# baowj-678/koordinator

Hardware: AMD Instinct MI355X
Metric: pods placed/sec + (pod,node) Filter+Score evals/sec at 50k nodes, 1-8 GPUs (higher is better)
Workload: dtype int64; 1 GPU; config4: 50000 nodes x 100000 pods, 30% BE, NodeResourcesFit + LoadAwareScheduling, shipped scheduler-config.yaml profile; nodes=50000, pods=100000, batch_pods=24, pipeline_lag=2, parallelism=node-shard x1

## Files before the change

### koordinator_amd/csrc/api.hip

```cpp
#include <hip/hip_runtime.h>
#include <rccl/rccl.h>

#include <algorithm>
#include <array>
#include <cmath>
#include <condition_variable>
#include <memory>
#include <mutex>
#include <cstdio>
#include <cstdlib>
#include <cstring>
#include <chrono>
#include <string>
#include <unordered_map>
#include <vector>

#include "../../include/koordhip.h"
#include "cls.h"
#include "diag.h"
#include "diag_ext.h"
#include "reasons.h"
#include "preempt.h"
#include "kernels.h"
#include "place_plan.hpp"
// ... 2541 lines not shown
  return 0;
}

int enqueue_rounds(koordhip_ctx *c, const PlaceCall &pc) {
  const kh::PlacePlan &plan = pc.plan;
  if (plan.cls) return 0;
  const int32_t P = plan.P, K = plan.K, lag = plan.lag, total = c->n_staged, lo = pc.lo, hi = pc.hi;
  const bool two = plan.two, exch = plan.exch, serial = plan.serial;
  kh::PipeSync *sync = pc.sync;
  hipStream_t rs = serial ? c->stream : c->rstream;
  for (int32_t r = 0; r < plan.rounds; r++) {
    const int32_t p0 = r * P, np = std::min(P, total - p0);
    const int par = r & 1;
    hipStream_t es = (two && par) ? c->stream2 : c->stream;
    const int slot = two ? par : 0;
    const kh::DevPod *pods = c->d_pods + p0;
    const bool timed = r % plan.tstride == 0;
    uint64_t *lists = c->d_lists + (size_t)(r & (2 * lag - 1)) * kListBuf;
    if (r > lag && !serial) HIP_TRY(kh::launch_wait_resolved(sync, r - lag, es));
    if (exch) {
      if (np < P) HIP_TRY(hipMemsetAsync(lists, 0, (size_t)P * K * sizeof(uint64_t), es));
      if (int e = topk_batch(c, pods, np, K, lo, hi, lists, timed, nullptr, 0, es, slot)) return e;
      if (int e = exchange(c, lists, (size_t)P * K, slot, es)) return e;
      HIP_TRY(kh::launch_topk_merge(gather_buf(c, slot), K, (int64_t)P * K, np, c->world, K, c->score_bits,
                                    c->d_final + (size_t)(r & (2 * lag - 1)) * kListBuf, sync, par, es));
    } else {
      if (int e = topk_batch(c, pods, np, K, lo, hi, lists, timed, sync, par, es, slot)) return e;
    }
    if (!plan.persistent) {
      if (!serial) {
        HIP_TRY(hipEventRecord(c->ev_res[r % kRing], c->stream));
        HIP_TRY(hipStreamWaitEvent(rs, c->ev_res[r % kRing], 0));
      }
      int32_t tm = -1;
      if (int e = timed_begin(c, TK_RESOLVE, rs, &tm)) return e;
      if (int e = launch_resolve_rounds(c, pc, r, r + 1, c->monotone, 1, rs)) return e;
      if (int e = timed_end(c, tm, rs)) return e;
    }
  }
  return 0;
}

int join_streams(koordhip_ctx *c, const PlaceCall &pc) {
  const kh::PlacePlan &plan = pc.plan;
  if (int e = timed_end(c, pc.res_tm, c->rstream)) return e;
  if (plan.two) {
    HIP_TRY(hipEventRecord(c->ev_eval2, c->stream2));
    HIP_TRY(hipStreamWaitEvent(c->stream, c->ev_eval2, 0));
  }
  if (plan.ext_pipe && plan.rounds > 0) {
    HIP_TRY(hipStreamWaitEvent(c->stream, c->ev_ext, 0));
    HIP_TRY(hipStreamWaitEvent(c->stream, c->ev_ext2, 0));
  }
  if (!plan.serial) {
    HIP_TRY(hipEventRecord(c->ev_res[0], c->rstream));
    HIP_TRY(hipStreamWaitEvent(c->stream, c->ev_res[0], 0));
  }
  HIP_TRY(hipEventRecord(c->t1, c->stream));
  c->pipe_check = true;
  return 0;
}

int print_stamps(koordhip_ctx *c, const kh::PlacePlan &plan) {
  if (!c->d_dbg) return 0;
  uint64_t h[64];
  HIP_TRY(hipMemcpyAsync(h, c->d_dbg, sizeof(h), hipMemcpyDeviceToHost, c->stream));
  HIP_TRY(hipStreamSynchronize(c->stream));
  if (c->eval_fused && h[40])
    std::fprintf(stderr,
                 "[koordhip stamps] k_eval_topk: %llu workgroups, cycles per workgroup: evaluate %.0f  select+emit %.0f  "
                 "publish %.0f | %llu merges, cycles per merge %.0f, candidates per merge %.1f\n",
                 (unsigned long long)h[40], (double)h[41] / h[40], (double)h[42] / h[40], (double)h[43] / h[40],
                 (unsigned long long)h[45], h[45] ? (double)h[44] / h[45] : 0.0, h[45] ? (double)h[46] / h[45] : 0.0);
  std::fprintf(stderr,
               "[koordhip stamps] resolve cycles: prologue walk %llu  hash %llu  waiting for lists %llu  loop %llu  "
               "release %llu | pods %llu  bulk commits %llu  staged pods %llu  general-path pods %llu  HBM row loads %llu\n",
               (unsigned long long)h[0], (unsigned long long)h[2], (unsigned long long)h[1], (unsigned long long)h[4],
               (unsigned long long)h[14], (unsigned long long)h[7], (unsigned long long)h[20],
               (unsigned long long)h[21], (unsigned long long)h[5], (unsigned long long)h[6]);
  std::fprintf(stderr, "[koordhip stamps] resolve loop cycles: conflict detection %llu  bulk commits %llu | "
               "general path: candidate+keys %llu  commit %llu | write-back %llu | kernel total %llu\n",
               (unsigned long long)h[16], (unsigned long long)h[17], (unsigned long long)h[18],
               (unsigned long long)h[19], (unsigned long long)h[25], (unsigned long long)h[26]);
  std::fprintf(stderr, "[koordhip stamps] round overlap: wave-0 end-of-round barrier %llu | wave 1: waiting for the "
               "next lists %llu  loading them %llu\n",
               (unsigned long long)h[29], (unsigned long long)h[27], (unsigned long long)h[28]);
  if (c->numa)
    std::fprintf(stderr, "[koordhip stamps] NUMA: accumulator replays full %llu cycles / %llu, spread %llu / %llu | "
                 "row passes of required-spread pods %llu / %llu, of other pods %llu / %llu\n",
                 (unsigned long long)h[32], (unsigned long long)h[33], (unsigned long long)h[34],
                 (unsigned long long)h[35], (unsigned long long)h[36], (unsigned long long)h[37],
                 (unsigned long long)h[38], (unsigned long long)h[39]);
  std::fprintf(stderr, "[koordhip stamps] general path detail: candidate + table keys %llu  row evaluations %llu | "
               "pods served by the key tables %llu\n",
               (unsigned long long)h[22], (unsigned long long)h[23], (unsigned long long)h[24]);
  std::fprintf(stderr, "[koordhip stamps] prologue phases: walk %llu  winner rows %llu (HBM loads %llu)  conflicts %llu | "
               "general-path causes: staged conflict %llu  slow %llu  voided by a general commit %llu\n",
               (unsigned long long)h[48], (unsigned long long)h[49], (unsigned long long)h[51],
               (unsigned long long)h[50], (unsigned long long)h[52], (unsigned long long)h[53],
               (unsigned long long)h[54]);
  std::fprintf(stderr, "[koordhip stamps] general path split: list + X + c %llu cycles | pods with ready key tables %llu | "
               "evaluation passes %llu\n",
               (unsigned long long)h[55], (unsigned long long)h[56], (unsigned long long)h[57]);
  if (plan.cls) {
    uint64_t q[32];
    HIP_TRY(hipMemcpy(q, c->d_dbg + 64, sizeof(q), hipMemcpyDeviceToHost));
    const double nl = (double)std::max<uint64_t>(q[7], 1), nc = (double)std::max<uint64_t>(q[15], 1);
    std::fprintf(stderr, "[koordhip stamps] class lists, cycles per launch (workgroup 0, %llu launches): buffer %.0f  log %.0f  "
                 "touched keys %.0f  compaction %.0f  sort %.0f  merge %.0f  outputs %.0f | builds (%llu): histogram %.0f  "
                 "fine %.0f  emit %.0f  sort %.0f  write %.0f\n", (unsigned long long)q[7], q[0] / nl, q[1] / nl, q[2] / nl,
                 q[3] / nl, q[4] / nl, q[5] / nl, q[6] / nl, (unsigned long long)q[15], q[8] / nc, q[9] / nc, q[10] / nc,
                 q[11] / nc, q[12] / nc);
  }
  {
    uint64_t q[4] = {0, 0, 0, 0}, rw[8] = {0, 0, 0, 0, 0, 0, 0, 0};
    HIP_TRY(hipMemcpy(q, c->d_dbg + 90, sizeof(q), hipMemcpyDeviceToHost));
    HIP_TRY(hipMemcpy(rw, c->d_dbg + 107, sizeof(rw), hipMemcpyDeviceToHost));
    std::fprintf(stderr, "[koordhip stamps] chain re-walks: walk + keys %llu (entries + claims %llu, row + evaluation "
                 "%llu)  winners' rows %llu cycles | winner rows loaded from HBM %llu\n", (unsigned long long)rw[0],
                 (unsigned long long)rw[5], (unsigned long long)rw[6], (unsigned long long)rw[1],
                 (unsigned long long)rw[2]);
    std::fprintf(stderr, "[koordhip stamps] chained decisions: %llu cycles, %llu pods resolved | claim tables %llu  "
                 "re-walks %llu  re-check + closure %llu  final table %llu | rounds with a lazy "
                 "claim table %llu\n", (unsigned long long)h[62],
                 (unsigned long long)h[63], (unsigned long long)q[0], (unsigned long long)q[1],
                 (unsigned long long)q[2], (unsigned long long)q[3], (unsigned long long)rw[7]);
    uint64_t sp[7] = {0, 0, 0, 0, 0, 0, 0};
    HIP_TRY(hipMemcpy(sp, c->d_dbg + 116, sizeof(sp), hipMemcpyDeviceToHost));
    std::fprintf(stderr, "[koordhip stamps] same-class speculation: made %llu  validated %llu  invalidated %llu | "
                 "given up: no head row %llu  walk past the entries %llu  winner assumed-claimed %llu  winner row in "
                 "HBM %llu\n", (unsigned long long)sp[0], (unsigned long long)sp[1], (unsigned long long)sp[2],
                 (unsigned long long)sp[3], (unsigned long long)sp[4], (unsigned long long)sp[5],
                 (unsigned long long)sp[6]);
  }
  if (plan.ext_pipe) {
    uint64_t q[8];
    HIP_TRY(hipMemcpy(q, c->d_dbg + 80, sizeof(q), hipMemcpyDeviceToHost));
    const double np = (double)std::max<uint64_t>(q[6], 1);
    std::fprintf(stderr, "[koordhip stamps] device pods (k_ext_pre / k_ext_final): %llu, resolve cycles from the "
                 "hand-off to the answer %llu (%.0f per pod) | final launch per pod: workgroup 0 evaluate + fold "
                 "%.0f | last workgroup: decide + publish %.0f  device commit %.0f\n",
                 (unsigned long long)h[31], (unsigned long long)h[30], h[31] ? (double)h[30] / h[31] : 0.0,
                 q[0] / np, q[3] / np, q[4] / np);
    uint64_t r[16];
    HIP_TRY(hipMemcpy(r, c->d_dbg + 96, sizeof(r), hipMemcpyDeviceToHost));
    std::fprintf(stderr, "[koordhip stamps] device-pod finals: workgroups with a full (device) re-evaluation %llu, "
                 "their re-evaluation %.2f us each\n", (unsigned long long)r[14], r[14] ? r[15] * 0.01 / r[14] : 0.0);
    const double nb = (double)std::max<uint64_t>(r[10], 1);
    std::fprintf(stderr, "[koordhip stamps] device-pod finals, us: request seen -> last workgroup arrived %.2f per pod | "
                 "per workgroup: -> gate seen %.2f  X marked %.2f  re-evaluated %.2f  folded + arrived %.2f\n",
                 r[5] * 0.01 / np, r[6] * 0.01 / nb, r[7] * 0.01 / nb, r[8] * 0.01 / nb, r[9] * 0.01 / nb);
    std::fprintf(stderr, "[koordhip stamps] device-pod hand-offs, us per pod: the request seen -> published %.2f | "
                 "requests already set when the final's first workgroup started: %llu of %llu | pre-evaluation "
                 "published after the request: %llu pods, waited %.2f us each\n",
                 r[2] * 0.01 / np, (unsigned long long)r[0], (unsigned long long)q[6], (unsigned long long)r[1],
                 r[1] ? r[3] * 0.01 / r[1] : 0.0);
  }
  std::fprintf(stderr, "[koordhip stamps] general commit split: row source %llu  Reserve delta %llu  voiding + "
               "outputs %llu cycles | winners already in M %llu\n",
               (unsigned long long)h[58], (unsigned long long)h[59], (unsigned long long)h[60],
               (unsigned long long)h[61]);
  return 0;
}

int place_staged_impl(koordhip_ctx *c) {
  if (!c->loaded) return fail(KOORDHIP_ESTATE, "no snapshot loaded");
  c->pipe_err = false;
  c->pipe_errc = 0;
  c->pipe_check = false;
// ... 1124 lines not shown
```

### koordinator_amd/csrc/eval.hpp

```cpp
#pragma once
#include <hip/hip_runtime.h>
#include <stdint.h>

#include "../../include/koordhip.h"
#include "numa.hpp"

namespace kh {

template <typename T>
__device__ __forceinline__ void st_wt(T *p, T v) {
  if constexpr (sizeof(T) == 8) {
    __hip_atomic_store(reinterpret_cast<uint64_t *>(p), __builtin_bit_cast(uint64_t, v), __ATOMIC_RELAXED,
                       __HIP_MEMORY_SCOPE_AGENT);
  } else if constexpr (sizeof(T) == 4) {
    __hip_atomic_store(reinterpret_cast<uint32_t *>(p), __builtin_bit_cast(uint32_t, v), __ATOMIC_RELAXED,
                       __HIP_MEMORY_SCOPE_AGENT);
  } else {
    __hip_atomic_store(reinterpret_cast<uint8_t *>(p), __builtin_bit_cast(uint8_t, v), __ATOMIC_RELAXED,
                       __HIP_MEMORY_SCOPE_AGENT);
  }
}

template <typename T>
using gptr = __attribute__((address_space(1))) T *;
// ... 573 lines not shown
  v.sa = d.sallow ? as_global(d.sallow)[i] : 0xFFFFFFFFu;
}

template <bool Z = true>
__device__ __forceinline__ void load_numa_row(NumaRow &r, const DevNodes &d, int32_t i) {
  r.cls = as_global(d.nu.node_cls)[i];
  r.nflags = as_global(d.nu.nflags)[i];
  r.cnt = as_global(d.nu.cnt)[i];
#pragma unroll
  for (int w = 0; w < NW; w++) {
    r.fr[w] = as_global(d.nu.fr[w])[i];
    r.ep[w] = as_global(d.nu.ep[w])[i];
    r.en[w] = as_global(d.nu.en[w])[i];
  }
  if (Z && d.nu.za && topo_policy(r.nflags) != 0) load_zones(r, d, i);
  r.amp = d.nu.amp ? as_global(d.nu.amp)[i] : 1.0;
}

template <bool Z = true>
__device__ __forceinline__ void store_numa_row(const NumaRow &r, const DevNodes &d, int32_t i) {
  d.nu.cnt[i] = r.cnt;
#pragma unroll
  for (int w = 0; w < NW; w++) {
    d.nu.fr[w][i] = r.fr[w];
    d.nu.ep[w][i] = r.ep[w];
    d.nu.en[w][i] = r.en[w];
  }
  if (Z && d.nu.za && topo_policy(r.nflags) != 0) {
    double *zu = d.nu.zu + (size_t)i * 2 * ZMAX;
#pragma unroll
    for (int q = 0; q < ZMAX; q++) {
      zu[q] = r.zu[0][q];
      zu[ZMAX + q] = r.zu[1][q];
    }
  }
}

__device__ __forceinline__ void numa_apply(NumaRow &r, const DevPod &p, const uint64_t *cpus, int sign,
                                           const uint64_t *P = nullptr) {
  const int ex = (int)KOORDHIP_NUMA_EXCLUSIVE(p.numa_policy);
  int n = 0;
#pragma unroll
  for (int w = 0; w < NW; w++) {
    n += __popcll(P ? (cpus[w] & ~P[w]) : cpus[w]);
    if (sign > 0) {
      r.fr[w] &= ~cpus[w];
      r.ep[w] = (r.ep[w] & ~cpus[w]) | (ex == (int)KOORDHIP_CPUEXCL_PCPU ? cpus[w] : 0ull);
      r.en[w] = (r.en[w] & ~cpus[w]) | (ex == (int)KOORDHIP_CPUEXCL_NUMA ? cpus[w] : 0ull);
    } else {
      r.fr[w] |= cpus[w];
      r.ep[w] &= ~cpus[w];
      r.en[w] &= ~cpus[w];
    }
  }
  r.cnt += sign * n;
}

__device__ __forceinline__ void store_row(const NV &v, const DevNodes &d, int32_t i) {
#pragma unroll
  for (int r = 0; r < KOORDHIP_NRES; r++) d.requested[r][i] = v.r[r];
  d.npods[i] = v.npods;
  d.nz_cpu[i] = v.nz_cpu;
  d.nz_mem[i] = v.nz_mem;
  d.la_used_cpu[i] = v.la_u_cpu;
  d.la_used_mem[i] = v.la_u_mem;
  d.la_used_prod_cpu[i] = v.la_up_cpu;
  d.la_used_prod_mem[i] = v.la_up_mem;
  d.flags[i] = (uint8_t)v.flags;
}

__device__ __forceinline__ void store_row_wt(const NV &v, const DevNodes &d, int32_t i) {
#pragma unroll
  for (int r = 0; r < KOORDHIP_NRES; r++) st_wt_g(&d.requested[r][i], v.r[r]);
  st_wt_g(&d.npods[i], v.npods);
  st_wt_g(&d.nz_cpu[i], v.nz_cpu);
  st_wt_g(&d.nz_mem[i], v.nz_mem);
  st_wt_g(&d.la_used_cpu[i], v.la_u_cpu);
  st_wt_g(&d.la_used_mem[i], v.la_u_mem);
  st_wt_g(&d.la_used_prod_cpu[i], v.la_up_cpu);
  st_wt_g(&d.la_used_prod_mem[i], v.la_up_mem);
  st_wt_g(&d.flags[i], (uint8_t)v.flags);
}

template <bool Z = true>
__device__ __forceinline__ void store_numa_row_wt(const NumaRow &r, const DevNodes &d, int32_t i) {
  st_wt_g(&d.nu.cnt[i], r.cnt);
#pragma unroll
  for (int w = 0; w < NW; w++) {
    st_wt_g(&d.nu.fr[w][i], r.fr[w]);
    st_wt_g(&d.nu.ep[w][i], r.ep[w]);
    st_wt_g(&d.nu.en[w][i], r.en[w]);
  }
  if (Z && d.nu.za && topo_policy(r.nflags) != 0) {
    double *zu = d.nu.zu + (size_t)i * 2 * ZMAX;
#pragma unroll
    for (int q = 0; q < ZMAX; q++) {
      st_wt_g(&zu[q], r.zu[0][q]);
      st_wt_g(&zu[ZMAX + q], r.zu[1][q]);
    }
  }
}

template <bool Z, bool WAVE = false>
__device__ __attribute__((noinline)) bool numa_reserve(const DevNumaClass *classes, NumaRow &row, const DevPod &pod,
                                                       uint64_t *cpus_out, const uint64_t *pref = nullptr) {
  NumaRow r = row;
  const DevPod p = pod;
  uint64_t cpus[NW] = {0, 0, 0, 0};
  uint64_t P[NW] = {0, 0, 0, 0};
  if (pref)
    for (int w = 0; w < NW; w++) P[w] = pref[w];
  for (int w = 0; w < NW; w++) cpus_out[w] = 0;
  const bool cs = (p.flags & KOORDHIP_POD_CPUSET) != 0;
  const int tp = Z ? topo_policy(r.nflags) : 0;
  if (!cs && tp == 0) return true;
  if (r.cls < 0) return false;
  const DevNumaClass &C = classes[r.cls];
  if (!Z || tp == 0) {
    if (cs && any4(P)) {
      if (!numa_allocate_pref_in<WAVE>(C, r, p, P, cpus)) return false;
    } else if (!numa_allocate_in<WAVE>(C, r, p, cpus)) {
      return false;
    }
    numa_apply(r, p, cpus, +1, P);
  } else {
    uint32_t mask;
    double av[2][ZMAX];
    zone_avail_all(r, C.nnuma, av);
    if (!zone_hint(C.nnuma, av, p, tp, &mask)) return false;
    const bool hp = cs && any4(P);
    if (hp) {
      double ru[ZMAX];
      zone_reusable(C, P, ru);
      zone_avail_reus(r, C.nnuma, ru, av);
    }
    double z[2][ZMAX];
    if (mask && !zone_alloc(C.nnuma, av, p, mask, z)) return false;
    if (cs) {
      if (mask) {
        if (!zone_allocate_in(C, r, p, z, cpus, hp ? P : nullptr)) return false;
      } else if (hp) {
        if (!numa_allocate_pref_in<WAVE>(C, r, p, P, cpus)) return false;
      } else if (!numa_allocate_in<WAVE>(C, r, p, cpus)) {
        return false;
      }
      numa_apply(r, p, cpus, +1, P);
    }
    if (mask) {
#pragma unroll
      for (int k = 0; k < ZMAX; k++) {
        r.zu[0][k] += z[0][k];
        r.zu[1][k] += z[1][k];
      }
    }
  }
  row = r;
  for (int w = 0; w < NW; w++) cpus_out[w] = cpus[w];
  return true;
}

template <int S>
__device__ __forceinline__ uint32_t filter_status(const DevCfg &c, const DevPod &pod, const NV &v,
                                                  const NumaRowRS<S> &r, const DevNumaClass *classes, int nmatch,
                                                  uint32_t mm, ResvXS rx = no_rx()) {
  uint32_t b = 0;
  if ((c.filt & KOORDHIP_PLUGIN_NODE_STATIC) && !((v.sa >> pod.sclass) & 1u)) b |= KOORDHIP_ST_STATIC_FAIL;
// ... 72 lines not shown
```

### koordinator_amd/csrc/kernels.hip

```cpp
#include <hip/hip_runtime.h>

#include <algorithm>
#include <cstdio>

#include "eval.hpp"
#include "karg.hpp"
#include "kernels.h"
#include "pipe.hpp"
#include "rows.hpp"

namespace kh {


__device__ __forceinline__ uint64_t shfl_u64(uint64_t v, int src) {
  uint32_t lo = __shfl((uint32_t)v, src, 64);
  uint32_t hi = __shfl((uint32_t)(v >> 32), src, 64);
  return ((uint64_t)hi << 32) | lo;
}
__device__ __forceinline__ uint64_t shfl_up_u64(uint64_t v, int d) {
  uint32_t lo = __shfl_up((uint32_t)v, d, 64);
  uint32_t hi = __shfl_up((uint32_t)(v >> 32), d, 64);
  return ((uint64_t)hi << 32) | lo;
}
__device__ __forceinline__ uint64_t shfl_xor_u64(uint64_t v, int m) {
// ... 1329 lines not shown
  NR *prenr2 = reinterpret_cast<NR *>(lds + ofs.pre_numa2);
  int32_t *pre_node2 = reinterpret_cast<int32_t *>(lds + ofs.pre_node2);
  __shared__ int32_t pnode[RES_MAXP_ROUND];
  __shared__ int32_t pgen[RES_MAXP_ROUND];
  __shared__ int32_t seg_w[RES_MAXP_ROUND];
  __shared__ int32_t ckey[RES_HASH], cval[RES_HASH];
  __shared__ int32_t sh_mp, sh_stop, sh_done, sh_chain;
  __shared__ uint64_t sh_rsv;
  const int t = threadIdx.x, lane = lane_id();
  const int32_t words = (n_nodes + 31) >> 5;
  const int32_t HP = max(1, RES_PRE / P);
  auto nodes = [&]() -> decltype(auto) {
    if constexpr (NM <= 2) {
      return *reinterpret_cast<const DevNodes *>(lds + ofs.ptab);
    } else {
      const DevNodes *p = dn;
      asm volatile("" : "+s"(p));
      return DevNodes(*p);
    }
  };
  if constexpr (NM <= 2) {
    constexpr int PW = (int)((NUMA ? offsetof(DevNodes, rv) : offsetof(DevNodes, nu)) / 8);
    static_assert(PW <= RES_THREADS, "one 8-byte word of the pointer table per thread");
    if (t < PW) reinterpret_cast<uint64_t *>(lds + ofs.ptab)[t] = reinterpret_cast<const uint64_t *>(dn)[t];
  }
  const bool two = kp > 64;
  const bool chain_on = (monotone & 2) && ofs.dep >= 0;
  static_assert(RES_WE == 8, "a pod's rank word: one rank byte + RES_WE - 1 predecessor bytes");
  const bool spec_on = NM == 0 && chain_on && ofs.rank >= 0 && pod_cls != nullptr && !(monotone & 16);
  uint64_t *rk = reinterpret_cast<uint64_t *>(lds + (ofs.rank >= 0 ? ofs.rank : 0));
  uint64_t *rk2 = reinterpret_cast<uint64_t *>(lds + (ofs.rank2 >= 0 ? ofs.rank2 : 0));
  const uint64_t t_kernel = (dbg && t == 0) ? stamp() : 0;
  if (t == 0) {
    sh_mp = r_begin > 0 ? min(mbuf[0], P) : 0;
    sh_stop = 0;
  }
  for (int32_t x = t; x < words; x += RES_THREADS) {
    modmap[x] = 0;
    gbits[x] = 0;
  }
  for (int32_t x = t; x < RES_MAXP_ROUND; x += RES_THREADS) {
    moved[x] = 0;
    ready[x] = 0;
  }
  for (int32_t x = t; x < RES_HASH; x += RES_THREADS) {
    ckey[x] = -1;
    cval[x] = 64;
  }
  const DevNumaClass *cls = ncls;
  if constexpr (NUMA) {
    const int32_t nc = dn->nu.ncls;
    if (nc <= NUMA_LDS_CLASSES) {
      uint4 *dst = reinterpret_cast<uint4 *>(lds + ofs.classes);
      const uint4 *src = reinterpret_cast<const uint4 *>(ncls);
      for (int32_t x = t; x < nc * (int32_t)(sizeof(DevNumaClass) / 16); x += RES_THREADS) dst[x] = src[x];
      cls = reinterpret_cast<const DevNumaClass *>(lds + ofs.classes);
    }
  }
  __syncthreads();
  if (t < sh_mp) {
    const int32_t nd = mbuf[1 + t];
    pnode[t] = nd;
    NV v;
    load_row(v, nodes(), nd);
    prow[t] = v;
    if constexpr (NUMA) {
      NR rr;
      load_side_row<NM>(rr, nodes(), nd);
      pnr[t] = rr;
    }
    atomicOr(&modmap[nd >> 5], 1u << (nd & 31));
  }
  __syncthreads();
  int32_t my_node = -1;
  auto word_doff = [](int q) -> int32_t {
    if (q >= 5 && q < 10) return (q - 5) * 8;
    if (q == 10 || q == 11) return (int32_t)offsetof(DevPod, nz_cpu_m) + (q - 10) * 8;
    if (q == 14 || q == 16) return (int32_t)offsetof(DevPod, est_cpu);
    if (q == 15 || q == 17) return (int32_t)offsetof(DevPod, est_mem);
    return -1;
  };
  const int32_t doff = word_doff(lane);
  uint64_t c_pro = 0, c_wait = 0, c_loop = 0, c_rel = 0, c_hash = 0, c_wb = 0;
  uint64_t c_w1wait = 0, c_w1load = 0, c_bar = 0;
  uint64_t c_l[4] = {0, 0, 0, 0};
  uint64_t n_slow = 0, n_miss = 0, n_staged = 0, n_bulk = 0, n_tab = 0;
  uint64_t c_g[2] = {0, 0};
  uint64_t c_nx[8] = {0, 0, 0, 0, 0, 0, 0, 0};
  uint64_t c_p[3] = {0, 0, 0}, n_p2 = 0, n_conf = 0, n_slowc = 0, n_void = 0;
  uint64_t c_cand = 0, n_evpass = 0, n_tready = 0;
  uint64_t c_gc[3] = {0, 0, 0}, n_ghit = 0;
  uint64_t c_chain = 0;
  uint64_t c_ch[4] = {0, 0, 0, 0};
  uint64_t c_rw[4] = {0, 0, 0, 0}, n_chbm = 0;
  uint64_t n_lazy = 0;
  uint64_t c_ext = 0, n_ext = 0;
  auto load_round = [&](int32_t rr, int32_t rp0, int32_t rn, uint64_t *Lk, DevPod *Lp, NV *Pr, NR *Pn,
                        int32_t *Pnode, uint64_t *Rk, int32_t tid, int32_t nth) {
    const uint64_t *L = lists0 + (size_t)(rr & (2 * lag - 1)) * list_buf;
    const int32_t tot = rn * k;
    const int32_t rl = t - 64;
    int32_t mycls = -1;
    if (Rk && rl >= 0 && rl < rn) mycls = pod_cls[rp0 + rl];
    uint64_t he[2] = {0, 0};
    bool hv[2];
#pragma unroll
    for (int u = 0; u < 2; u++) {
      const int32_t sl = tid + u * nth, j = sl / HP, q = sl - j * HP;
      hv[u] = sl < RES_PRE && j < rn && q < k;
      if (u * nth < RES_PRE) he[u] = L[min(j * k + q, tot - 1)];
    }
    constexpr int LB = 6;
    const uint4 *L4 = reinterpret_cast<const uint4 *>(L);
    const int32_t n16 = (tot + 1) >> 1;
    auto put = [&](int32_t e, uint64_t v) {
      if (e < tot) {
        const int32_t j = e / k, q = e - j * k;
        Lk[j * kp + q] = v;
      }
    };
    auto put2 = [&](int32_t x, const uint4 &w) {
      if (x < n16) {
        put(2 * x, ((uint64_t)w.y << 32) | w.x);
        put(2 * x + 1, ((uint64_t)w.w << 32) | w.z);
      }
    };
    uint4 lv[LB];
#pragma unroll
    for (int u = 0; u < LB; u++)
      if (u * nth < n16) lv[u] = L4[min(tid + u * nth, n16 - 1)];
    const uint4 *psrc = reinterpret_cast<const uint4 *>(pods + rp0);
    uint4 *pdst = reinterpret_cast<uint4 *>(Lp);
    const int32_t p16 = rn * (int32_t)(sizeof(DevPod) / 16);
    uint4 a0, a1, a2, a3;
    a0 = psrc[min(tid, p16 - 1)];
    if (nth < p16) a1 = psrc[min(tid + nth, p16 - 1)];
    if (2 * nth < p16) a2 = psrc[min(tid + 2 * nth, p16 - 1)];
    if (3 * nth < p16) a3 = psrc[min(tid + 3 * nth, p16 - 1)];
    int32_t nd[2];
    NV v[2];
#pragma unroll
    for (int u = 0; u < 2; u++) {
      nd[u] = (hv[u] && he[u] != 0) ? key_node(he[u]) : -1;
      if (u * nth < RES_PRE)
        if (nd[u] >= 0) load_row(v[u], nodes(), nd[u]);
    }
    for (int32_t b = 0;;) {
      const int32_t nb = b + LB * nth;
      const bool more = nb < n16;
      uint4 nx[LB];
      if (more) {
#pragma unroll
        for (int u = 0; u < LB; u++)
          if (nb + u * nth < n16) nx[u] = L4[min(nb + tid + u * nth, n16 - 1)];
      }
#pragma unroll
      for (int u = 0; u < LB; u++) put2(b + tid + u * nth, lv[u]);
      if (!more) break;
#pragma unroll
      for (int u = 0; u < LB; u++) lv[u] = nx[u];
      b = nb;
    }
    for (int32_t x = tid; x < rn * (kp - k); x += nth) {
      const int32_t j = x / (kp - k), q = k + x - j * (kp - k);
      Lk[j * kp + q] = 0ull;
    }
// ... 2 lines not shown
    if (tid + 2 * nth < p16) pdst[tid + 2 * nth] = a2;
    if (tid + 3 * nth < p16) pdst[tid + 3 * nth] = a3;
    for (int32_t b = 4 * nth; b < p16; b += 4 * nth) {
      const int32_t x0 = b + tid, x1 = x0 + nth, x2 = x0 + 2 * nth, x3 = x0 + 3 * nth;
      const uint4 c0 = psrc[min(x0, p16 - 1)], c1 = psrc[min(x1, p16 - 1)], c2 = psrc[min(x2, p16 - 1)],
                  c3 = psrc[min(x3, p16 - 1)];
      if (x0 < p16) pdst[x0] = c0;
      if (x1 < p16) pdst[x1] = c1;
      if (x2 < p16) pdst[x2] = c2;
      if (x3 < p16) pdst[x3] = c3;
    }
#pragma unroll
    for (int u = 0; u < 2; u++) {
      const int32_t sl = tid + u * nth;
      if (sl >= RES_PRE) continue;
      if (nd[u] >= 0) {
        Pr[sl] = v[u];
        if constexpr (NUMA) {
          NR rr2;
          load_side_row<NM>(rr2, nodes(), nd[u]);
          Pn[sl] = rr2;
        }
      }
      Pnode[sl] = nd[u];
    }
    for (int32_t sl = tid + 2 * nth; sl < RES_PRE; sl += nth) {
      const int32_t j = sl / HP, q = sl - j * HP;
      int32_t n1 = -1;
      if (j < rn && q < k) {
        const uint64_t e = L[(size_t)j * k + q];
        if (e != 0) n1 = key_node(e);
      }
      if (n1 >= 0) {
        NV v1;
        load_row(v1, nodes(), n1);
        Pr[sl] = v1;
        if constexpr (NUMA) {
          NR rr2;
          load_side_row<NM>(rr2, nodes(), n1);
          Pn[sl] = rr2;
        }
      }
      Pnode[sl] = n1;
    }
    if (Rk && rl >= 0 && rl < 64) {
      uint64_t w = 0;
      int32_t cnt = 0;
      for (int32_t j = 0; j < rn; j++) {
        const int32_t cj = __builtin_amdgcn_readlane(mycls, j);
        if (j < rl && cj == mycls) {
          if (cnt < RES_WE - 1) w |= (uint64_t)j << (8 * (cnt + 1));
          cnt++;
        }
      }
      if (rl < rn) Rk[rl] = w | (uint64_t)cnt;
    }
  };
  auto prev_slot = [&](int32_t nd) -> int32_t {
    uint32_t h = res_hash(nd);
    for (;;) {
      const int32_t x = hnode[h];
      if (x == nd) return hslot[h];
      if (x < 0) return -1;
      h = (h + 1) & (RES_HASH - 1);
    }
  };
  for (int32_t r = r_begin, p0 = r_begin * P; r < r_end && p0 < total; r++, p0 += P) {
    const int32_t n_pods = min(P, total - p0);
    const bool preloaded = ofs.overlap && r > r_begin;
    const uint64_t t_w0 = (dbg && t == 0) ? stamp() : 0;
    if (!preloaded) {
      if (t == 0 && !wait_at_least(&sy->sel[r & 1], P * (r >> 1) + n_pods, sy)) sh_stop = 1;
      __syncthreads();
    }
    if (sh_stop) return;
    const uint64_t t_entry = (dbg && t == 0) ? stamp() : 0;
    const int32_t mp = sh_mp;
    if (!preloaded) {
      const bool first = r == r_begin;
      load_round(r, p0, n_pods, lk, lpod, pre, prenr, pre_node, (spec_on && !first) ? rk : nullptr, t, RES_THREADS);
      if (spec_on && first)
        for (int32_t x = t; x < n_pods; x += RES_THREADS) rk[x] = 0ull;
    }
    for (int32_t x = t; x < RES_HASH; x += RES_THREADS) hnode[x] = -1;
    if (t == 0) {
      sh_done = 0;
      sh_chain = 0;
    }
    __syncthreads();
    if (t < mp) {
      const int32_t nd = pnode[t];
      uint32_t h = res_hash(nd);
      while (atomicCAS(&hnode[h], -1, nd) != -1) h = (h + 1) & (RES_HASH - 1);
      hslot[h] = t;
    }
    __syncthreads();
    const uint64_t t_a = (dbg && t == 0) ? stamp() : 0;
    if (mp > 0 && t < RES_PRE) {
      const int32_t nd = pre_node[t];
      if (nd >= 0 && prev_slot(nd) >= 0) pre_node[t] = -1;
    }
    for (int32_t base = 0; base < n_pods * RES_WE; base += RES_THREADS) {
      const int32_t x = base + t;
      const int32_t l = x / RES_WE, q = x - l * RES_WE;
      const bool live = l < n_pods;
      const uint64_t e = (live && q < kp) ? lk[l * kp + q] : 0ull;
      const int32_t nd = e ? key_node(e) : -1;
      const bool inx = e != 0 && xbit(modmap, nd);
      const int g = lane & ~(RES_WE - 1);
      const uint32_t bx = (uint32_t)(__ballot(live && e != 0 && !inx) >> g) & 0xFFu;
      const uint32_t bz = (uint32_t)(__ballot(live && e == 0) >> g) & 0xFFu;
      const int f = bx ? __builtin_ctz(bx) : RES_WE, z = bz ? __builtin_ctz(bz) : RES_WE;
      const bool general = f == RES_WE && z == RES_WE;
      bool spec = false;
      int fw = f, gu = -1;
      uint64_t rkw = 0;
      if constexpr (NM == 0) {
        if (spec_on) {
          rkw = live ? rk[l] : 0ull;
          const int rank = (int)(rkw & 0xFFull);
          if (rank > 0 && !(lpod[l].flags & KH_POD_EXT)) {
            uint32_t b = bx;
            for (int u = 0; u < rank && b; u++) b &= b - 1u;
            if (rank < RES_WE && b && __builtin_ctz(b) < z) {
              spec = true;
              fw = __builtin_ctz(b);
            } else {
              gu = 1;
            }
          }
          if (__ballot(spec)) {
            const bool nohead = spec && q < fw && !inx && !(q < HP && pre_node[l * HP + q] == nd);
            if (spec && ((uint32_t)(__ballot(nohead) >> g) & 0xFFu)) {
              spec = false;
              fw = f;
              gu = 0;
            }
          }
        }
      }
      bool walked = live && !general && (q < min(fw, z) || (q == fw && fw < z));
      bool assumed = spec && q < fw && !inx;
      uint64_t key = 0;
      int32_t ms = -1;
      if (walked) {
        if (q < min(fw, z)) {
          const DevPod pod = lpod[l];
          NV v;
          if (assumed) {
            v = pre[l * HP + q];
            apply_delta(v, pod, +1);
          } else {
            ms = prev_slot(nd);
            v = slot_row(prow[ms]);
          }
          key = make_key(eval_row<NM>(pod, v, pnr[ms >= 0 ? ms : 0], cls, c), nd);
        } else {
          key = e;
        }
      }
      uint64_t mx = key;
#pragma unroll
      for (int m = 1; m < RES_WE; m <<= 1) {
        const uint64_t o = shfl_xor_u64(mx, m);
        mx = o > mx ? o : mx;
      }
      if constexpr (NM == 0) {
        if (__ballot(spec)) {
          const bool win = spec && walked && key == mx && mx != 0;
          const uint32_t brep = (uint32_t)(__ballot(win && assumed) >> g) & 0xFFu;
          const uint32_t bhbm =
              (uint32_t)(__ballot(win && q == fw && !(q < HP && pre_node[l * HP + q] == nd)) >> g) & 0xFFu;
          const bool back = spec && (brep | bhbm) != 0u;
          if (back) {
            spec = false;
            gu = brep ? 2 : 3;
            fw = f;
            assumed = false;
            walked = q < min(f, z) || (q == f && f < z);
// ... 696 lines not shown
          }
          if (!okr) {
            result = KOORDHIP_RESERVE_FAILED;
          } else {
            result = w;
            const uint64_t xw = lane < RES_WORDS ? reinterpret_cast<const uint64_t *>(srow)[lane] : 0ull;
            const double dq = (doff >= 0 && (lane < 16 || ((prodmask >> g) & 1ull)))
                                  ? *reinterpret_cast<const double *>(reinterpret_cast<const char *>(&lpod[g]) + doff)
                                  : 0.0;
            uint64_t x = xw;
            if (lane < 18) x = (uint64_t)__double_as_longlong(__longlong_as_double((long long)xw) + dq);
            if (lane == 18) x += 1ull << 32;
            if (lane < RES_WORDS) reinterpret_cast<uint64_t *>(&mrow[rw])[lane] = x;
            if (lane == 0) atomicOr(&gbits[w >> 5], 1u << (w & 31));
            if (!hit) {
              if (lane == rw) my_node = w;
              gvalid |= 1ull << rw;
              if (lane == 0) {
                atomicOr(&modmap[w >> 5], 1u << (w & 31));
                if (from_prev >= 0) moved[from_prev] = 1;
              }
              nm++;
            }
            gclap(1);
            bool met = false;
#pragma unroll
            for (int q = 0; q < RES_WE; q++) met = met || se[q] == w;
            uint64_t voided = __ballot(lane > g && met);
            for (;;) {
              const uint64_t nx = __ballot(lane > g && ((ok >> lane) & 1ull) && !((voided >> lane) & 1ull) &&
                                           (mydep & voided) != 0ull);
              if (!nx) break;
              voided |= nx;
            }
            if (dbg) n_void += __popcll(ok & voided);
            ok &= ~voided;
          }
        }
        if (lane == 0) st_wt(&out_node[p0 + g], result);
        if (out_cpus && lane < NW)
          out_cpus[(size_t)(p0 + g) * NW + lane] =
              lane == 0 ? cpus[0] : (lane == 1 ? cpus[1] : (lane == 2 ? cpus[2] : cpus[3]));
        gclap(2);
        lap(3);
        j = g + 1;
      }
      const uint64_t t_wb = dbg ? stamp() : 0;
      if (lane < nm && ((lazy >> lane) & 1ull)) {
        const int32_t pi = seg_p[lane];
        my_node = seg_w[lane];
        const int32_t src = dec_src[pi];
        const uint64_t *sr = reinterpret_cast<const uint64_t *>(src >= 0 ? &pre[src] : &prow[-src - 1]);
        uint64_t *dr = reinterpret_cast<uint64_t *>(&mrow[lane]);
        const char *pp = reinterpret_cast<const char *>(&lpod[pi]);
        const bool prod = ((prodmask >> pi) & 1ull) != 0;
#pragma unroll
        for (int h = 0; h < 2; h++) {
          uint64_t x[RES_WORDS / 2];
          double dq[RES_WORDS / 2];
#pragma unroll
          for (int u = 0; u < RES_WORDS / 2; u++) {
            const int q = h * (RES_WORDS / 2) + u;
            const int32_t o = word_doff(q);
            x[u] = sr[q];
            dq[u] = (o >= 0 && (q < 16 || prod)) ? *reinterpret_cast<const double *>(pp + o) : 0.0;
          }
#pragma unroll
          for (int u = 0; u < RES_WORDS / 2; u++) {
            const int q = h * (RES_WORDS / 2) + u;
            uint64_t y = x[u];
            if (word_doff(q) >= 0) y = (uint64_t)__double_as_longlong(__longlong_as_double((long long)y) + dq[u]);
            if (q == 18) y += 1ull << 32;
            dr[q] = y;
          }
        }
        if constexpr (NUMA) {
          const uint64_t *sn = reinterpret_cast<const uint64_t *>(src >= 0 ? &prenr[src] : &pnr[-src - 1]);
          uint64_t *dn2 = reinterpret_cast<uint64_t *>(&mnr[lane]);
#pragma unroll 4
          for (int w = 0; w < (int)(sizeof(NR) / 8); w++) dn2[w] = sn[w];
        }
      }
      if (lane < nm) {
        const NV v = slot_row(mrow[lane]);
        mrow[lane] = v;
        store_row_wt(v, nodes(), my_node);
        if constexpr (NUMA) {
          const NR nr = mnr[lane];
          store_side_row_wt<NM>(nr, nodes(), my_node);
        }
      }
      if (lane == 0) __hip_atomic_store(&sh_done, 1, __ATOMIC_RELAXED, __HIP_MEMORY_SCOPE_WORKGROUP);
      const bool surv = lag > 1 && lane < mp && pgen[lane] == r - 1 && !moved[lane];
      const uint64_t sbm = __ballot(surv);
      const int32_t ns = __popcll(sbm);
      const int32_t sidx = nm + __popcll(sbm & ((1ull << lane) - 1ull));
      int32_t snode = -1;
      if (surv) {
        snode = pnode[lane];
        mrow[sidx] = prow[lane];
        if constexpr (NUMA) mnr[sidx] = pnr[lane];
      }
      if (lane < mp) modmap[pnode[lane] >> 5] = 0;
      if (lane < nm) {
        modmap[my_node >> 5] = 0;
        gbits[my_node >> 5] = 0;
      }
      for (int32_t x = lane; x < RES_HASH; x += 64) {
        ckey[x] = -1;
        cval[x] = 64;
      }
      if (lane < nm) {
        atomicOr(&modmap[my_node >> 5], 1u << (my_node & 31));
        pnode[lane] = my_node;
        pgen[lane] = r;
      }
      if (surv) {
        atomicOr(&modmap[snode >> 5], 1u << (snode & 31));
        pnode[sidx] = snode;
        pgen[sidx] = r - 1;
      }
      moved[lane] = 0;
      const uint64_t t_rel = dbg ? stamp() : 0;
      if (dbg) c_wb += t_rel - t_wb;
      if (lane == 0) {
        sh_mp = nm + ns;
        asm volatile("s_waitcnt vmcnt(0)" ::: "memory");
        __hip_atomic_store(&sy->res_round, r + 1, __ATOMIC_RELAXED, __HIP_MEMORY_SCOPE_AGENT);
      }
      if (dbg) {
        const uint64_t t_end = stamp();
        c_rel += t_end - t_rel;
        c_loop += t_end - t_loop;
      }
    } else if (t < 64 * (1 + res_loaders<NM>())) {
      if (ofs.overlap && r + 1 < r_end && p0 + P < total) {
        const int32_t np2 = min(P, total - (p0 + P));
        int ok = 1;
        const uint64_t t1 = dbg ? stamp() : 0;
        if (lane == 0) ok = wait_at_least(&sy->sel[(r + 1) & 1], P * ((r + 1) >> 1) + np2, sy) ? 1 : 0;
        const uint64_t t2 = dbg ? stamp() : 0;
        if (__builtin_amdgcn_readfirstlane(ok)) {
          load_round(r + 1, p0 + P, np2, lk2, lpod2, pre2, prenr2, pre_node2, spec_on ? rk2 : nullptr, t - 64,
                     64 * res_loaders<NM>());
          if (dbg) {
            asm volatile("s_waitcnt vmcnt(0) lgkmcnt(0)" ::: "memory");
            c_w1load += stamp() - t2;
          }
        } else if (lane == 0) {
          sh_stop = 1;
        }
        if (dbg) c_w1wait += t2 - t1;
      }
    } else {
      const int hw = __builtin_amdgcn_readfirstlane((t >> 6) - 1 - res_loaders<NM>()),
                nh = RES_THREADS / 64 - 1 - res_loaders<NM>();
      if (chain_on)
        while (!__hip_atomic_load(&sh_chain, __ATOMIC_ACQUIRE, __HIP_MEMORY_SCOPE_WORKGROUP)) __builtin_amdgcn_s_sleep(1);
      uint64_t todo = __ballot(lane < n_pods && dec_c[lane] == 1);
      for (int32_t x = 0; x < hw && todo; x++) todo &= todo - 1ull;
      for (; have_tables && todo;) {
        const int32_t l = (int32_t)__builtin_ctzll(todo);
        for (int32_t x = 0; x < nh && todo; x++) todo &= todo - 1ull;
        if (__hip_atomic_load(&sh_done, __ATOMIC_RELAXED, __HIP_MEMORY_SCOPE_WORKGROUP)) break;
        const DevPod pod = uniform_pod(lpod[l]);
        for (int32_t b0 = 0; b0 < l + mp; b0 += 64) {
          const int32_t x = b0 + lane;
          int32_t v = 0;
          if (x < l) {
            const uint64_t kk = dec_key[x];
            if (kk != 0 && dec_n[x] >= 0) {
              const int32_t src = dec_src[x];
              NV row = src >= 0 ? pre[src] : prow[-src - 1];
              NR nr;
              if constexpr (NUMA) nr = src >= 0 ? prenr[src] : pnr[-src - 1];
              const DevPod pi = lpod[x];
              apply_delta(row, pi, +1);
              v = eval_row<NM>(pod, row, nr, cls, c) + 1;
            }
            kput(kpre, l * RES_MAXP_ROUND + x, (uint32_t)v);
          } else if (x < l + mp) {
            const int32_t sl = x - l;
            NR nr;
            if constexpr (NUMA) nr = pnr[sl];
            v = eval_row<NM>(pod, slot_row(prow[sl]), nr, cls, c) + 1;
            kput(ktab, l * RES_MAXP_ROUND + sl, (uint32_t)v);
          }
        }
        if (lane == 0) __hip_atomic_store(&ready[l], 1, __ATOMIC_RELEASE, __HIP_MEMORY_SCOPE_WORKGROUP);
      }
    }
    const uint64_t t_bar = (dbg && t == 0) ? stamp() : 0;
    __syncthreads();
    if (dbg && t == 0) c_bar += stamp() - t_bar;
    for (int32_t x = t; x < RES_MAXP_ROUND; x += RES_THREADS) ready[x] = 0;
    if (ofs.overlap) {
      uint64_t *a = lk;
      lk = lk2;
      lk2 = a;
      DevPod *b = lpod;
      lpod = lpod2;
      lpod2 = b;
      NV *c2 = pre;
      pre = pre2;
      pre2 = c2;
      NR *d2 = prenr;
      prenr = prenr2;
      prenr2 = d2;
      int32_t *e2 = pre_node;
      pre_node = pre_node2;
      pre_node2 = e2;
      uint64_t *f2 = rk;
      rk = rk2;
      rk2 = f2;
    }
    {
      NV *x = prow;
      prow = mrow;
      mrow = x;
      NR *y = pnr;
      pnr = mnr;
      mnr = y;
    }
  }
  if (t <= RES_MAXP_ROUND && t <= sh_mp) mbuf[t] = t == 0 ? sh_mp : pnode[t - 1];
  if (dbg && n_p2) atomicAdd((unsigned long long *)&dbg[51], (unsigned long long)n_p2);
  if (dbg && n_evpass) atomicAdd((unsigned long long *)&dbg[57], (unsigned long long)n_evpass);
  if (dbg && t == 64) {
    atomicAdd((unsigned long long *)&dbg[27], (unsigned long long)c_w1wait);
    atomicAdd((unsigned long long *)&dbg[28], (unsigned long long)c_w1load);
  }
  if (dbg && t == 0) {
    atomicAdd((unsigned long long *)&dbg[0], (unsigned long long)c_pro);
    atomicAdd((unsigned long long *)&dbg[1], (unsigned long long)c_wait);
    atomicAdd((unsigned long long *)&dbg[2], (unsigned long long)c_hash);
    atomicAdd((unsigned long long *)&dbg[4], (unsigned long long)c_loop);
    atomicAdd((unsigned long long *)&dbg[5], (unsigned long long)n_slow);
    atomicAdd((unsigned long long *)&dbg[6], (unsigned long long)n_miss);
    atomicAdd((unsigned long long *)&dbg[7], (unsigned long long)total);
    atomicAdd((unsigned long long *)&dbg[14], (unsigned long long)c_rel);
    atomicAdd((unsigned long long *)&dbg[25], (unsigned long long)c_wb);
    atomicAdd((unsigned long long *)&dbg[26], (unsigned long long)(stamp() - t_kernel));
    atomicAdd((unsigned long long *)&dbg[29], (unsigned long long)c_bar);
    for (int q = 0; q < 8; q++) atomicAdd((unsigned long long *)&dbg[32 + q], (unsigned long long)c_nx[q]);
    for (int q = 0; q < 4; q++) atomicAdd((unsigned long long *)&dbg[16 + q], (unsigned long long)c_l[q]);
    atomicAdd((unsigned long long *)&dbg[20], (unsigned long long)n_bulk);
    atomicAdd((unsigned long long *)&dbg[21], (unsigned long long)n_staged);
    atomicAdd((unsigned long long *)&dbg[22], (unsigned long long)c_g[0]);
    atomicAdd((unsigned long long *)&dbg[24], (unsigned long long)n_tab);
    atomicAdd((unsigned long long *)&dbg[23], (unsigned long long)c_g[1]);
    for (int q = 0; q < 3; q++) atomicAdd((unsigned long long *)&dbg[48 + q], (unsigned long long)c_p[q]);
    atomicAdd((unsigned long long *)&dbg[52], (unsigned long long)n_conf);
    atomicAdd((unsigned long long *)&dbg[53], (unsigned long long)n_slowc);
    atomicAdd((unsigned long long *)&dbg[54], (unsigned long long)n_void);
    atomicAdd((unsigned long long *)&dbg[55], (unsigned long long)c_cand);
    atomicAdd((unsigned long long *)&dbg[56], (unsigned long long)n_tready);
    atomicAdd((unsigned long long *)&dbg[58], (unsigned long long)c_gc[0]);
    atomicAdd((unsigned long long *)&dbg[59], (unsigned long long)c_gc[1]);
    atomicAdd((unsigned long long *)&dbg[60], (unsigned long long)c_gc[2]);
    atomicAdd((unsigned long long *)&dbg[61], (unsigned long long)n_ghit);
    atomicAdd((unsigned long long *)&dbg[62], (unsigned long long)c_chain);
    for (int q = 0; q < 4; q++) atomicAdd((unsigned long long *)&dbg[90 + q], (unsigned long long)c_ch[q]);
    atomicAdd((unsigned long long *)&dbg[107], (unsigned long long)c_rw[0]);
    atomicAdd((unsigned long long *)&dbg[108], (unsigned long long)c_rw[1]);
    atomicAdd((unsigned long long *)&dbg[109], (unsigned long long)n_chbm);
    atomicAdd((unsigned long long *)&dbg[112], (unsigned long long)c_rw[2]);
    atomicAdd((unsigned long long *)&dbg[113], (unsigned long long)c_rw[3]);
    atomicAdd((unsigned long long *)&dbg[114], (unsigned long long)n_lazy);
    atomicAdd((unsigned long long *)&dbg[30], (unsigned long long)c_ext);
    atomicAdd((unsigned long long *)&dbg[31], (unsigned long long)n_ext);
  }
}


__global__ void k_commit(DevCfg c, DevNodes d, const DevPod *__restrict__ pod, int32_t node, int32_t sign,
                         uint64_t *__restrict__ cpus, int32_t *__restrict__ rc) {
  if (threadIdx.x != 0 || blockIdx.x != 0) return;
  const DevPod p = *pod;
  *rc = 0;
  NumaRowR8 rv{};
  if (c.resv) {
    load_resv(rv, d.rv, node);
    if (sign < 0 && resv_matchable(rv, p)) {
      *rc = KOORDHIP_EINVAL;
      return;
    }
  }
  uint64_t m[NW] = {0, 0, 0, 0};
  if (numa_on(c) && numa_active(p, c)) {
    NumaRow r;
    load_numa_row(r, d, node);
    if (sign > 0) {
      uint64_t pref[NW];
      resv_pref_cpus(rv, p, (c.resv && (c.score & KOORDHIP_PLUGIN_RESERVATION)) ? resv_matched(rv, p) : 0u, pref);
      if (!numa_reserve<true>(d.nu.cls, r, p, m, pref)) {
        *rc = KOORDHIP_ERESERVE;
        return;
      }
    } else if (topo_policy(r.nflags) != 0) {
      *rc = KOORDHIP_EINVAL;
      return;
    } else if (is_cpuset(p)) {
      for (int w = 0; w < NW; w++) m[w] = cpus[w];
      numa_apply(r, p, m, sign);
    }
    store_numa_row(r, d, node);
    if (sign > 0)
      for (int w = 0; w < NW; w++) cpus[w] = m[w];
  } else if (sign > 0) {
    for (int w = 0; w < NW; w++) cpus[w] = 0;
  }
  if (c.resv && sign > 0) {
    resv_assume(rv, p, m);
    store_resv(rv, d.rv, node);
  }
  NV v;
  load_row(v, d, node);
  apply_delta(v, p, sign);
// ... 346 lines not shown
```

Measured before the change: 1.852 million pods/s.

## Build next round's node hash in wave 0 and streamline row write-back

The node-to-slot hash table is now built only once at the first round. Later rounds get it from wave 0 at the end of the previous round, from the modified and surviving nodes, which removes a full-block clear, a hash pass and one barrier per round. The write-back now recomputes the overflow flags from raw row words and stores through pointers preloaded into registers, avoiding repeated struct pointer loads. This relies on wave 0's hash matching exactly what the old per-round rebuild produced, so correctness is more fragile. A new debug stamp counter is added as well.

```diff
diff --git a/koordinator_amd/csrc/api.hip b/koordinator_amd/csrc/api.hip
--- a/koordinator_amd/csrc/api.hip
+++ b/koordinator_amd/csrc/api.hip
@@ -2647,9 +2647,10 @@
                "general path: candidate+keys %llu  commit %llu | write-back %llu | kernel total %llu\n",
                (unsigned long long)h[16], (unsigned long long)h[17], (unsigned long long)h[18],
                (unsigned long long)h[19], (unsigned long long)h[25], (unsigned long long)h[26]);
-  std::fprintf(stderr, "[koordhip stamps] round overlap: wave-0 end-of-round barrier %llu | wave 1: waiting for the "
-               "next lists %llu  loading them %llu\n",
-               (unsigned long long)h[29], (unsigned long long)h[27], (unsigned long long)h[28]);
+  std::fprintf(stderr, "[koordhip stamps] round overlap: wave-0 end-of-round barrier %llu  next hash %llu | "
+               "wave 1: waiting for the next lists %llu  loading them %llu\n",
+               (unsigned long long)h[29], (unsigned long long)h[3], (unsigned long long)h[27],
+               (unsigned long long)h[28]);
   if (c->numa)
     std::fprintf(stderr, "[koordhip stamps] NUMA: accumulator replays full %llu cycles / %llu, spread %llu / %llu | "
                  "row passes of required-spread pods %llu / %llu, of other pods %llu / %llu\n",
diff --git a/koordinator_amd/csrc/eval.hpp b/koordinator_amd/csrc/eval.hpp
--- a/koordinator_amd/csrc/eval.hpp
+++ b/koordinator_amd/csrc/eval.hpp
@@ -679,6 +679,40 @@
   st_wt_g(&d.flags[i], (uint8_t)v.flags);
 }
 
+struct RowWtPtrs {
+  uint64_t p[13];
+};
+__device__ __forceinline__ RowWtPtrs load_row_wt_ptrs(const DevNodes &d) {
+  static_assert(KOORDHIP_NRES == 5 && offsetof(DevNodes, requested) == 48 && offsetof(DevNodes, nz_cpu) == 88 &&
+                    offsetof(DevNodes, npods) == 104 && offsetof(DevNodes, la_used_cpu) == 128 &&
+                    offsetof(DevNodes, la_used_prod_mem) == 152 && offsetof(DevNodes, flags) == 160,
+                "the pointer words load_row_wt_ptrs reads");
+  const uint4 *q = reinterpret_cast<const uint4 *>(&d);
+  const uint4 w0 = q[3], w1 = q[4], w2 = q[5], w3 = q[6], w4 = q[8], w5 = q[9];
+  const uint2 w6 = *reinterpret_cast<const uint2 *>(reinterpret_cast<const char *>(&d) + 160);
+  auto lo = [](const uint4 &w) { return ((uint64_t)w.y << 32) | w.x; };
+  auto hi = [](const uint4 &w) { return ((uint64_t)w.w << 32) | w.z; };
+  RowWtPtrs o;
+  o.p[0] = lo(w0), o.p[1] = hi(w0), o.p[2] = lo(w1), o.p[3] = hi(w1), o.p[4] = lo(w2), o.p[5] = hi(w2);
+  o.p[6] = lo(w3), o.p[7] = hi(w3), o.p[8] = lo(w4), o.p[9] = hi(w4), o.p[10] = lo(w5), o.p[11] = hi(w5);
+  o.p[12] = ((uint64_t)w6.y << 32) | w6.x;
+#pragma unroll
+  for (int i = 0; i < 13; i++) asm volatile("" : "+v"(o.p[i]));
+  return o;
+}
+__device__ __forceinline__ void store_row_wt(const NV &v, uint32_t flags, const RowWtPtrs &c, int32_t i) {
+#pragma unroll
+  for (int r = 0; r < KOORDHIP_NRES; r++) st_wt_g(reinterpret_cast<double *>(c.p[r]) + i, v.r[r]);
+  st_wt_g(reinterpret_cast<int32_t *>(c.p[7]) + i, v.npods);
+  st_wt_g(reinterpret_cast<double *>(c.p[5]) + i, v.nz_cpu);
+  st_wt_g(reinterpret_cast<double *>(c.p[6]) + i, v.nz_mem);
+  st_wt_g(reinterpret_cast<double *>(c.p[8]) + i, v.la_u_cpu);
+  st_wt_g(reinterpret_cast<double *>(c.p[9]) + i, v.la_u_mem);
+  st_wt_g(reinterpret_cast<double *>(c.p[10]) + i, v.la_up_cpu);
+  st_wt_g(reinterpret_cast<double *>(c.p[11]) + i, v.la_up_mem);
+  st_wt_g(reinterpret_cast<uint8_t *>(c.p[12]) + i, (uint8_t)flags);
+}
+
 template <bool Z = true>
 __device__ __forceinline__ void store_numa_row_wt(const NumaRow &r, const DevNodes &d, int32_t i) {
   st_wt_g(&d.nu.cnt[i], r.cnt);
diff --git a/koordinator_amd/csrc/kernels.hip b/koordinator_amd/csrc/kernels.hip
--- a/koordinator_amd/csrc/kernels.hip
+++ b/koordinator_amd/csrc/kernels.hip
@@ -1435,6 +1435,7 @@
   };
   const int32_t doff = word_doff(lane);
   uint64_t c_pro = 0, c_wait = 0, c_loop = 0, c_rel = 0, c_hash = 0, c_wb = 0;
+  uint64_t c_nh = 0;
   uint64_t c_w1wait = 0, c_w1load = 0, c_bar = 0;
   uint64_t c_l[4] = {0, 0, 0, 0};
   uint64_t n_slow = 0, n_miss = 0, n_staged = 0, n_bulk = 0, n_tab = 0;
@@ -1603,19 +1604,23 @@
       if (spec_on && first)
         for (int32_t x = t; x < n_pods; x += RES_THREADS) rk[x] = 0ull;
     }
-    for (int32_t x = t; x < RES_HASH; x += RES_THREADS) hnode[x] = -1;
+    const bool first_round = r == r_begin;
+    if (first_round)
+      for (int32_t x = t; x < RES_HASH; x += RES_THREADS) hnode[x] = -1;
     if (t == 0) {
       sh_done = 0;
       sh_chain = 0;
     }
-    __syncthreads();
-    if (t < mp) {
-      const int32_t nd = pnode[t];
-      uint32_t h = res_hash(nd);
-      while (atomicCAS(&hnode[h], -1, nd) != -1) h = (h + 1) & (RES_HASH - 1);
-      hslot[h] = t;
-    }
-    __syncthreads();
+    if (!preloaded) __syncthreads();
+    if (first_round) {
+      if (t < mp) {
+        const int32_t nd = pnode[t];
+        uint32_t h = res_hash(nd);
+        while (atomicCAS(&hnode[h], -1, nd) != -1) h = (h + 1) & (RES_HASH - 1);
+        hslot[h] = t;
+      }
+      __syncthreads();
+    }
     const uint64_t t_a = (dbg && t == 0) ? stamp() : 0;
     if (mp > 0 && t < RES_PRE) {
       const int32_t nd = pre_node[t];
@@ -2478,12 +2483,37 @@
         }
       }
       if (lane < nm) {
-        const NV v = slot_row(mrow[lane]);
-        mrow[lane] = v;
-        store_row_wt(v, nodes(), my_node);
+        const auto &d = nodes();
+        const uint64_t *mw = reinterpret_cast<const uint64_t *>(&mrow[lane]);
+        uint64_t w[RES_WORDS];
+#pragma unroll
+        for (int q = 0; q < RES_WORDS; q++)
+          if (q < 3 || (q >= 5 && q < 12) || q >= 14) w[q] = mw[q];
+#pragma unroll
+        for (int q = 0; q < RES_WORDS; q++)
+          if (q < 3 || (q >= 5 && q < 12) || q >= 14) asm volatile("" : "+v"(w[q]));
+        auto wd = [&](int q) { return __longlong_as_double((long long)w[q]); };
+        NV m;
+#pragma unroll
+        for (int q = 0; q < KOORDHIP_NRES; q++) m.r[q] = wd(5 + q);
+        m.nz_cpu = wd(10), m.nz_mem = wd(11);
+        m.la_u_cpu = wd(14), m.la_u_mem = wd(15), m.la_up_cpu = wd(16), m.la_up_mem = wd(17);
+        m.npods = (int32_t)(w[18] >> 32);
+        uint32_t f = (uint32_t)w[19] & ~(uint32_t)(NF_OVER_CPU | NF_OVER_MEM | NF_OVER_EPH);
+        if (m.r[KOORDHIP_RES_CPU] > wd(KOORDHIP_RES_CPU)) f |= NF_OVER_CPU;
+        if (m.r[KOORDHIP_RES_MEM] > wd(KOORDHIP_RES_MEM)) f |= NF_OVER_MEM;
+        if (m.r[KOORDHIP_RES_EPH] > wd(KOORDHIP_RES_EPH)) f |= NF_OVER_EPH;
+        mrow[lane].flags = f;
+        m.flags = f;
+        if constexpr (NM <= 2) {
+          const RowWtPtrs cp = load_row_wt_ptrs(d);
+          store_row_wt(m, f, cp, my_node);
+        } else {
+          store_row_wt(m, d, my_node);
+        }
         if constexpr (NUMA) {
           const NR nr = mnr[lane];
-          store_side_row_wt<NM>(nr, nodes(), my_node);
+          store_side_row_wt<NM>(nr, d, my_node);
         }
       }
       if (lane == 0) __hip_atomic_store(&sh_done, 1, __ATOMIC_RELAXED, __HIP_MEMORY_SCOPE_WORKGROUP);
@@ -2517,6 +2547,19 @@
         pgen[sidx] = r - 1;
       }
       moved[lane] = 0;
+      auto build_next_hash = [&]() {
+        if (r + 1 < r_end && p0 + P < total) {
+          for (int32_t x = lane; x < RES_HASH; x += 64) hnode[x] = -1;
+          wsync();
+          auto put_hash = [&](int32_t nd, int32_t slot) {
+            uint32_t h = res_hash(nd);
+            while (atomicCAS(&hnode[h], -1, nd) != -1) h = (h + 1) & (RES_HASH - 1);
+            hslot[h] = slot;
+          };
+          if (lane < nm) put_hash(my_node, lane);
+          if (surv) put_hash(snode, sidx);
+        }
+      };
       const uint64_t t_rel = dbg ? stamp() : 0;
       if (dbg) c_wb += t_rel - t_wb;
       if (lane == 0) {
@@ -2524,9 +2567,12 @@
         asm volatile("s_waitcnt vmcnt(0)" ::: "memory");
         __hip_atomic_store(&sy->res_round, r + 1, __ATOMIC_RELAXED, __HIP_MEMORY_SCOPE_AGENT);
       }
+      const uint64_t t_nh = dbg ? stamp() : 0;
+      build_next_hash();
       if (dbg) {
         const uint64_t t_end = stamp();
-        c_rel += t_end - t_rel;
+        c_rel += t_nh - t_rel;
+        c_nh += t_end - t_nh;
         c_loop += t_end - t_loop;
       }
     } else if (t < 64 * (1 + res_loaders<NM>())) {
@@ -2630,6 +2676,7 @@
     atomicAdd((unsigned long long *)&dbg[0], (unsigned long long)c_pro);
     atomicAdd((unsigned long long *)&dbg[1], (unsigned long long)c_wait);
     atomicAdd((unsigned long long *)&dbg[2], (unsigned long long)c_hash);
+    atomicAdd((unsigned long long *)&dbg[3], (unsigned long long)c_nh);
     atomicAdd((unsigned long long *)&dbg[4], (unsigned long long)c_loop);
     atomicAdd((unsigned long long *)&dbg[5], (unsigned long long)n_slow);
     atomicAdd((unsigned long long *)&dbg[6], (unsigned long long)n_miss);
```

Measured after the change: 1.857 million pods/s, median of 6. About the same (+0.3%).
